# brodeau/aerobulk

Measured on NVIDIA B200. Metric: grid points/s (FP64), higher is better.
Workload: dtype f64

## Files before the change

### aerobulk_b200/csrc/ab_device.cuh

```cuda
#pragma once

#include <cuda_runtime.h>
#include <math.h>

#include "ab_math.cuh"

namespace abd {

#ifndef AB_CS_UNROLL
#define AB_CS_UNROLL 1
#endif
constexpr int CS_UNROLL = AB_CS_UNROLL;
#ifndef AB_PASS_UNROLL
#define AB_PASS_UNROLL 1
#endif
constexpr int PASS_UNROLL = AB_PASS_UNROLL;
#define ABD __device__ __forceinline__
#if defined(AB_NOINLINE) && AB_NOINLINE
#define ABD_HEAVY static __device__ __noinline__
#else
#define ABD_HEAVY __device__ __forceinline__
#endif

template <unsigned long long B>
// ... 274 lines not shown
    } else {
        const PsiMH r = psi_mh_coare_unstable(zeta_u);
        m_u = r.m;
        h_u = r.h;
        if (!ZTEQ) h_t = psi_h_coare_unstable(zeta_t);
    }
}

ABD double cap_zeta(double zeta) { return abm::dmin(abm::dmax(zeta, -50.), 5.); }
ABD PsiMH psi_mh_ecmwf_stable(double zeta)
{
    constexpr double zc = 5. / 0.35;
    const double z = cap_zeta(zeta);
    const double t = KC(2. / 3.) * (z - KC(zc)) * abm::dexp_b(KC(-0.35) * z);
    const double a = fabs(1. + KC(2. / 3.) * z);
    PsiMH r;
    r.m = -t - z - KC(2. / 3. * zc);
    r.h = -t - a * abm::fast_sqrt_pos(a) - KC(2. / 3. * zc) + 1.;
    return r;
}
ABD PsiMH psi_mh_ecmwf_unstable(double zeta)
{
    const double z = cap_zeta(zeta);
    const double x2 = abm::fast_sqrt_pos(fabs(1. - 16. * z));
    const double x = abm::fast_sqrt_pos(x2);
    const double t = 1. + x;
    PsiMH r;
    r.m = abm::dlog(0.125 * t * t * (1. + x2)) - 2. * abm::datan_ge1(x) + KC(0.5 * RPI);
    r.h = 2. * abm::dlog(0.5 * (1. + x2));
    return r;
}
ABD double psi_m_ecmwf_stable(double zeta) { return psi_mh_ecmwf_stable(zeta).m; }
ABD double psi_h_ecmwf_stable(double zeta) { return psi_mh_ecmwf_stable(zeta).h; }
ABD double psi_m_ecmwf_unstable(double zeta) { return psi_mh_ecmwf_unstable(zeta).m; }
ABD double psi_h_ecmwf_unstable(double zeta)
{
    const double x2 = abm::fast_sqrt_pos(fabs(1. - 16. * cap_zeta(zeta)));
    return 2. * abm::dlog(0.5 * (1. + x2));
}

constexpr double ATAN_A_STABLE = 0x1.b53ea749504d7p-1;
constexpr double LOG_A_STABLE = -0x1.ecc2caec5160ap+0;
ABD double psi_m_andreas_stable(double zeta)
{
    const double z = abm::dmin(zeta, 15.);
    constexpr double zam = 5.;
    const double x = abm::fast_cbrt(fabs(1. + z));
    return -(KC(3. * zam / ZBM_A) * (x - 1.))
           + KC(zam * ZBBM_A / (2. * ZBM_A))
                 * (2. * abm::dlog(fabs((x + KC(ZBBM_A)) * KC(1. / (1. + ZBBM_A))))
                    - abm::dlog(fabs((x * x - x * KC(ZBBM_A) + KC(ZBBM_A * ZBBM_A)) * KC(1. / (1. - ZBBM_A + ZBBM_A * ZBBM_A))))
                    + KC(2. * SR3) * (abm::datan_ge1((2. * x - KC(ZBBM_A)) * KC(1. / (SR3 * ZBBM_A))) - KC(ATAN_A_STABLE)));
}
ABD double psi_h_andreas_stable(double zeta)
{
    const double z = abm::dmin(zeta, 15.);
    constexpr double zah = 5., zbh = 5., zch = 3.;
    const double zz = 2. * z + zch;
    return -(KC(0.5 * zbh) * abm::dlog(fabs(1. + zch * z + z * z)))
           + KC(-zah / SR5 + 0.5 * zbh * zch / SR5)
                 * (abm::dlog(fabs(fdiv(zz - KC(SR5), zz + KC(SR5)))) - KC(LOG_A_STABLE));
}
ABD PsiMH psi_mh_andreas_unstable(double zeta)
{
    const double z = abm::dmin(zeta, 15.);
    const double x2 = abm::dmax(abm::fast_sqrt_pos(fabs(1. - 16. * z)), 1.);
    const double x = abm::fast_sqrt_pos(x2);
    PsiMH r;
    const double l2 = abm::dlog(0.5 * (1. + x2));
    r.m = 2. * abm::dlog((1. + x) * 0.5) + l2 - 2. * abm::datan_ge1(x) + KC(RPI * 0.5);
    r.h = 2. * l2;
    return r;
}
ABD double psi_h_andreas_unstable(double zeta)
{
    const double x2 = abm::dmax(abm::fast_sqrt_pos(fabs(1. - 16. * abm::dmin(zeta, 15.))), 1.);
    return 2. * abm::dlog(0.5 * (1. + x2));
}

struct Uniform {
    double zt, zu;
    double log_zt, log_zu, log_ztu, log_zu10, log_10;
    double fg_c_a;
    double fg_1_o_Ribcu;
    double rdt, gdept;
    int nb_iter;
    unsigned long long wl_commit_mask;
    int isd;
    int dawn;
};

struct Guess {
    double us, ts, qs, t_zu, q_zu, Ub, z0;
};

template <bool ZTEQ>
ABD Guess first_guess_coare(const Uniform &u, double sst, double t_zt, double ssq, double q_zt, double wnd, double charn)
{
    Guess g;
    g.t_zu = abm::dmax(t_zt, 180.);
    g.q_zu = abm::dmax(q_zt, 1.e-6);

    double dt = floor_abs(g.t_zu - sst, 1.E-09);
    double dq = floor_abs(g.q_zu - ssq, 1.E-12);

    const double nu_a = visc_air(g.t_zu);
    const double Ub = sqrt(wnd * wnd + 0.5 * 0.5);
    double us = u.fg_c_a * Ub;

    double z0 = charn * us * us * INV_GRAV + fdiv(0.11 * nu_a, us);
    z0 = abm::dmin(abm::dmax(fabs(z0), 1.E-8), 1.);
    const double log_z0 = abm::dlog(z0);

    const double sq = fdiv(VKARMN, u.log_zu - log_z0);
    const double Cd = sq * sq;
    const double r1_o_sqrt_Cd10 = (u.log_10 - log_z0) * INV_VKARMN;

    const double log_z0t = abm::dmin(abm::dmax(u.log_10 - fdiv(VKARMN, 0.00115 * r1_o_sqrt_Cd10), LOG_1EM8), 0.);

    const double Rib = ri_bulk(u.zu, sst, g.t_zu, ssq, g.q_zu, Ub);

    const double cc = fdiv(VKARMN2, Cd * (u.log_zt - log_z0t));
    const double cc_ri = cc * Rib;
    const double zeta_u = nonneg(Rib) ? (cc_ri + 27. / 9. * Rib * Rib) : fdiv(cc_ri, 1. + Rib * u.fg_1_o_Ribcu);

    const double zeta_t = ZTEQ ? zeta_u : fdiv(u.zt * zeta_u, u.zu);
    double psi_m_u, psi_h_u, psi_h_t;
    psi3_coare<ZTEQ>(zeta_u, zeta_t, psi_m_u, psi_h_u, psi_h_t);
    us = abm::dmax(fdiv(Ub * VKARMN, u.log_zu - log_z0 - psi_m_u), 1.E-9);
    const double tmp = fdiv(VKARMN, u.log_zu - log_z0t - psi_h_u);
    double ts = dt * tmp;
    double qs = dq * tmp;

    if (!ZTEQ) {
        const double prf = u.log_ztu + psi_h_u - psi_h_t;
        g.t_zu = t_zt - ts * INV_VKARMN * prf;
        g.q_zu = q_zt - qs * INV_VKARMN * prf;
        g.q_zu = signbit(g.q_zu) ? 0. : g.q_zu;
        dt = floor_abs(g.t_zu - sst, 1.E-09);
        dq = floor_abs(g.q_zu - ssq, 1.E-12);
        ts = dt * tmp;
        qs = dq * tmp;
    }
    g.us = us;
    g.ts = ts;
    g.qs = qs;
    g.Ub = Ub;
    z0 = charn * us * us * INV_GRAV + fdiv(0.11 * nu_a, us);
    g.z0 = abm::dmin(abm::dmax(fabs(z0), 1.E-8), 1.);
    return g;
}

template <bool COARE_FORM>
ABD double cool_skin_dT(double alpha, double Qsw, double Qnsol, double us, double Qlat)
{
    const double usw = abm::dmax(us, KC(1.E-4)) * KC(SQ_RADRW);
    const double usw2 = usw * usw;
    const double c_lamb = fdiv(alpha * KC(RCST_CS), usw2 * usw2);
    const double nu_o_usw = fdiv(KC(RNU0_W), usw);
    const double d_warm = abm::dmin(6. * nu_o_usw, KC(0.007));
    const double q_lat_term = COARE_FORM ? fdiv(KC(0.026) * abm::dmin(Qlat, 0.) * KC(RCP0_W * (1. / RLEVAP)), alpha) : 0.;

    auto delta = [&](double Qd) -> double {
        const double zQd = COARE_FORM ? Qd + q_lat_term : Qd;
        if (nonneg(zQd)) return d_warm;
        const double x = abm::dmax(c_lamb * zQd, KC(1.e-30));
        const double x75 = abm::pow075_pos(x);
        return 6. * abm::fast_rcbrt(1. + x75) * nu_o_usw;
    };

    double Qabs = Qnsol, d = 0.;
#pragma unroll CS_UNROLL
    for (int jc = 0; jc < 5; ++jc) {
        const double d_prev = d;
        if (jc > 0) {
            const double fr = abm::dmax((COARE_FORM ? KC(0.137) : KC(0.065)) + 11. * d - fdiv(KC(6.6E-5), d) * (1. - abm::dexp(-d * KC(1. / 8.E-4))), KC(0.01));
            Qabs = Qnsol + fr * Qsw;
        }
        d = delta(Qabs);
        if (jc > 0 && d == d_prev) break;
    }
    return Qabs * d * KC(1. / RK0_W);
}

struct WarmLayer {
    double dT, Hz, Qac, Tac;
};

struct WlCoareCtx {
    double cd1, cd2;
    bool dawn;
};
__host__ __device__ inline bool wl_coare_dawn(double lon, int isd)
{
    auto f_mod = [](double a, double p) {
        double r = fmod(a, p);
        if (r != 0. && ((r < 0.) != (p < 0.))) r += p;
        return r;
    };
    double lag = -1. * f_mod((360. - f_mod(lon, 360.)) / 15., 24.);
    lag = -1. * copysign(fmin(fabs(lag), fabs(f_mod(lag, 24.))), lag + 12.);
    const int ilag = (int)(lag * 3600.);
    int isol = (isd + ilag) % 86400;
    if (isol < 0) isol += 86400;
    const double hr = (double)isol / 3600.;
    return (hr > 4.) && (hr <= 6.5);
}
ABD WlCoareCtx wl_coare_ctx(double alpha, bool dawn)
{
    WlCoareCtx c;
    c.dawn = dawn;
    const double Rich0 = 0.65;
    c.cd1 = sqrt(2. * Rich0 * RCP0_W / (alpha * GRAV * RHO0_W));
    c.cd2 = sqrt(2. * alpha * GRAV / (Rich0 * RHO0_W)) / RCP0W_POW15;
    return c;
}
ABD double wl_coare_absorption(double H)
{
    const double e1 = (H > KC(0.53)) ? 0. : abm::dexp_b(-H * KC(1. / 0.014));
    const double e2 = (H > KC(13.4)) ? 0. : abm::dexp_b(-H * KC(1. / 0.357));
    return 1. - fdiv(KC(0.28 * 0.014) * (1. - e1) + KC(0.27 * 0.357) * (1. - e2)
                     + KC(0.45 * 12.82) * (1 - abm::dexp_b(-H * KC(1. / 12.82))), H);
}
ABD void wl_coare(WarmLayer &w, const WlCoareCtx &c, double Qsw, double Qnsol, double Tau, double rdt,
                  double gdept, bool commit)
{
    const double Hwl_max = 20.;
    double dT = w.dT;
    double H = abm::dmax(abm::dmin(w.Hz, Hwl_max), 0.1);
    double qac = w.Qac;
    double tac = w.Tac;
    bool l_exit = c.dawn, destroy = c.dawn;
    double Qabs = 0.;

    if (!l_exit) {
        Qabs = wl_coare_absorption(H) * Qsw + Qnsol;
        if (fabs(dT) < 1.E-6 && Qabs <= 0.) l_exit = true;
    }
    if (!l_exit && (w.Qac + Qabs * rdt <= 0.)) {
        l_exit = true;
        destroy = true;
    }
    if (!l_exit) {
        tac = w.Tac + abm::dmax(.002, Tau) * rdt;
#pragma unroll 1
        for (int jl = 0; jl < 5; ++jl) {
            if (jl > 0) Qabs = wl_coare_absorption(H) * Qsw + Qnsol;
            qac = w.Qac + Qabs * rdt;
            if (qac <= 0.) break;
            const double H_prev = H;
            H = abm::dmax(abm::dmin(Hwl_max, c.cd1 * tac * abm::fast_rsqrt(qac)), 0.1);
            if (H == H_prev) break;
        }
        if (qac <= 0.) {
            destroy = true;
        } else {
            dT = fdiv(c.cd2 * (qac * (qac * abm::fast_rsqrt(qac))), tac);
            if (signbit(gdept - H)) dT = dT * fdiv(gdept, H);
        }
    }
    if (destroy) {
        dT = 0.;
        H = Hwl_max;
        qac = 0.;
        tac = 0.;
    }
    if (commit) {
        w.dT = dT;
        w.Hz = H;
        w.Qac = qac;
        w.Tac = tac;
    }
}

ABD double phi_takaya(double z)
{
    const double z2 = z * z;
    if (nonneg(z)) return 1. + fdiv(5. * z + 4. * z2, 1. + 3. * z + 0.25 * z2);
    return abm::fast_rsqrt(1. - 16. * (-fabs(z)));
}
struct WlEcmwfCtx {
    double fr, tcorr, r_tcorr;
};
ABD WlEcmwfCtx wl_ecmwf_ctx(double H, double gdept)
{
    WlEcmwfCtx c;
    c.tcorr = signbit(gdept - H) ? gdept / H : 1.;
    c.r_tcorr = 1. / c.tcorr;
    c.fr = 1. - 0.28 * abm::dexp(-71.5 * H) - 0.27 * abm::dexp(-2.8 * H) - 0.45 * abm::dexp(-0.07 * H);
    return c;
}
ABD void wl_ecmwf(WarmLayer &w, const WlEcmwfCtx &c, double alpha, double Qsw, double Qnsol, double us, double rdt)
{
    const double rNuwl0 = 0.5;
    const double RhoCp_w = RHO0_W * RCP0_W;
    const double H = w.Hz;
    const double tcorr = c.tcorr;
    const double dT_b = abm::dmax(w.dT * c.r_tcorr, 0.);

    const double Qabs = c.fr * Qsw + Qnsol;

    const double usw = abm::dmax(us, KC(1.E-4)) * KC(SQ_RADRW);
    const double usw2 = usw * usw;
    const bool warming = nonneg(Qabs);

    const double cst1 = KC(VKARMN * GRAV) * alpha;
    const double L2 = fdiv(cst1 * Qabs, RhoCp_w * usw2 * usw);
    const double cst2 = fdiv(cst1, 5. * H * usw2);
    const double cst0 = fdiv(rdt * (rNuwl0 + 1.), H);
    const double A = cst0 * Qabs * KC(1. / (rNuwl0 * RhoCp_w));
    const double cst3 = -cst0 * KC(VKARMN) * usw * KC(FLA_ECMWF);

    const double B_warm = warming ? fdiv(cst3, phi_takaya(H * L2)) : 0.;
    double dT_n = dT_b;
#pragma unroll 2
    for (int jc = 0; jc < 10; ++jc) {
        const double prev = dT_n;
        dT_n = 0.5 * (dT_n + dT_b);
        const double B = warming ? B_warm : fdiv(cst3, phi_takaya(H * abm::fast_sqrt(dT_n * cst2)));
        dT_n = abm::dmax(dT_b + A + B * dT_n, 0.);
        if (dT_n == prev) break;
    }
    w.dT = dT_n * tcorr;
}

struct PointIn {
    double sst, theta_zt, ssq, q_zt, wnd, slp;
    double Qsw, rlw, lon;
    bool has_lon;
};
struct Coeffs {
    double Cd, Ch, Ce, t_zu, q_zu, Ub, Ts, qs;
};
struct Diag {
    double CdN, ChN, CeN, z0, us, L, UN10, dT_cs;
};

ABD double cd_n10_ncar(double w)
{
    double w6 = w * w * w;
    w6 = w6 * w6;
    const double r = nonneg(w - 33.) ? KC(1.e-3 * 2.34)
                                     : KC(1.e-3) * (fdiv(KC(2.7), w) + KC(0.142) + w * KC(1. / 13.09) - KC(3.14807E-10) * w6);
    return abm::dmax(r, KC(CX_MIN));
}

template <bool ZTEQ>
ABD Coeffs solve_ncar(const Uniform &u, const PointIn &p, Diag &dg)
{
    const double Ub = abm::dmax(0.5, p.wnd);
    const bool stable0 = nonneg(virt_temp(p.theta_zt, p.q_zt) - virt_temp(p.sst, p.ssq));
    double CdN = cd_n10_ncar(Ub);
    double sqrt_CdN = abm::fast_sqrt_pos(CdN);
    double Cd = CdN;
    double Ce = abm::dmax(1.e-3 * (34.6 * sqrt_CdN), CX_MIN);
    double Ch = abm::dmax(1.e-3 * sqrt_CdN * (stable0 ? 18. : 32.7), CX_MIN);
    double sqrt_Cd = sqrt_CdN;
    double t_zu = abm::dmax(p.theta_zt, 180.);
    double q_zu = abm::dmax(p.q_zt, 1.e-6);
    double us = 0., r1oL = 0., Un10 = 0., ChN = 0., CeN = 0.;

#pragma unroll 1
    for (int jit = 0; jit < u.nb_iter; ++jit) {
        const double dt = t_zu - p.sst;
        const double dq = q_zu - p.ssq;
        us = sqrt_Cd * Ub;
        const double r_sqrt_Cd = abm::fast_rcp(sqrt_Cd);
        const double ts = Ch * r_sqrt_Cd * dt;
        const double qs = Ce * r_sqrt_Cd * dq;
        r1oL = one_on_L(t_zu, q_zu, us, ts, qs);
        const double zeta_u = clip_abs(u.zu * r1oL, 10.);
        const double zeta_t = clip_abs(u.zt * r1oL, 10.);
        double psi_m, psi_h_u, psi_h_t = 0.;
        if (nonneg(zeta_u)) {
            psi_m = psi_h_u = -5. * zeta_u;
            if (!ZTEQ) psi_h_t = -5. * zeta_t;
        } else {
            const PsiMH r = psi_mh_ncar_unstable(zeta_u);
            psi_m = r.m;
            psi_h_u = r.h;
            if (!ZTEQ) psi_h_t = psi_h_ncar_unstable(zeta_t);
        }
        if (!ZTEQ) {
            const double tmp = u.log_ztu + psi_h_u - psi_h_t;
            t_zu = p.theta_zt - ts * INV_VKARMN * tmp;
            q_zu = abm::dmax(0., p.q_zt - qs * INV_VKARMN * tmp);
        }
        Un10 = abm::dmax(0.25, sqrt_Cd * Ub * INV_VKARMN * (VKARMN * r_sqrt_Cd + psi_m - u.log_zu10));
        CdN = cd_n10_ncar(Un10);
        sqrt_CdN = abm::fast_sqrt_pos(CdN);
        double tmp = 1. + sqrt_CdN * INV_VKARMN * (u.log_zu10 - psi_m);
        Cd = abm::dmax(fdiv(CdN, tmp * tmp), CX_MIN);
        sqrt_Cd = abm::fast_sqrt_pos(Cd);
        const double r_sqrt_CdN = abm::fast_rcp(sqrt_CdN);
        tmp = (u.log_zu10 - psi_h_u) * INV_VKARMN * r_sqrt_CdN;
        const double tmp2 = sqrt_Cd * r_sqrt_CdN;
        ChN = 1.e-3 * sqrt_CdN * (nonneg(zeta_u) ? 18. : 32.7);
        CeN = 1.e-3 * (34.6 * sqrt_CdN);
        Ch = abm::dmax(fdiv(ChN * tmp2, 1. + ChN * tmp), CX_MIN);
        Ce = abm::dmax(fdiv(CeN * tmp2, 1. + CeN * tmp), CX_MIN);
    }
    Coeffs c;
    c.Cd = Cd; c.Ch = Ch; c.Ce = Ce; c.t_zu = t_zu; c.q_zu = q_zu; c.Ub = Ub; c.Ts = p.sst; c.qs = p.ssq;
    dg.CdN = CdN; dg.ChN = ChN; dg.CeN = CeN; dg.UN10 = Un10; dg.L = 1. / r1oL; dg.us = us;
    dg.z0 = abm::dmin(u.zu * abm::dexp_b(-VKARMN * abm::fast_rsqrt(CdN)), Z0_SEA_MAX);
    dg.dT_cs = 0.;
    return c;
}

ABD double charn_coare3p0(double w)
{
    if (!nonneg(w - 10.)) return 0.011;
    if (nonneg(w - 18.)) return 0.018;
    return 0.011 + (0.018 - 0.011) * (w - 10.) * (1. / (18. - 10.));
}
ABD double charn_coare3p6(double w) { return abm::dmax(abm::dmin(KC(0.0017) * w - KC(0.005), KC(0.028)), 0.); }

template <bool V36, bool CS, bool WL, bool ZTEQ>
ABD Coeffs solve_coare(const Uniform &u, const PointIn &p, WarmLayer &wl, Diag &dg)
{
    constexpr bool SKIN = CS || WL;
    constexpr double zi0 = 600., Beta0 = V36 ? 1.2 : 1.25, zeta_abs_max = 50.;

    double Ts = p.sst, qs_ = p.ssq;
    double alpha = 0.;
    WlCoareCtx wc = {};
    if (SKIN) {
        if (CS) Ts = Ts - 0.25;
        qs_ = RDCT_QSAT_SALT * q_sat(abm::dmax(Ts, 200.), p.slp);
        alpha = alpha_sw(p.sst);
        if (WL) wc = wl_coare_ctx(alpha, p.has_lon ? wl_coare_dawn(p.lon, u.isd) : (u.dawn != 0));
    }

    const Guess g = first_guess_coare<ZTEQ>(u, Ts, p.theta_zt, qs_, p.q_zt, p.wnd,
                                            V36 ? charn_coare3p6(p.wnd) : charn_coare3p0(p.wnd));
    double us = g.us, ts = g.ts, qst = g.qs, t_zu = g.t_zu, q_zu = g.q_zu, Ub = g.Ub;
    double log_z0 = abm::dlog(g.z0);
    const double nu_a = V36 ? visc_air(t_zu) : visc_air(p.theta_zt);

    double dt = floor_abs(t_zu - Ts, 1.E-09);
    double dq = floor_abs(q_zu - qs_, 1.E-12);
    double dT_cs = 0., r1oL = 0., z0 = g.z0, log_z0t = 0.;

#pragma unroll 1
    for (int jit = 1; jit <= u.nb_iter; ++jit) {
        const double us2 = us * us;
        r1oL = one_on_L(t_zu, q_zu, us, ts, qst);

        const double cv = abm::fast_cbrt(abm::dmax(KC(-zi0 * INV_VKARMN) * r1oL, 0.));
        const double gust2 = KC(Beta0 * Beta0) * us2 * (cv * cv);
        Ub = abm::dmax(abm::fast_sqrt(p.wnd * p.wnd + gust2), KC(0.2));

        const double zeta_u = clip_abs(u.zu * r1oL, zeta_abs_max);

        const double Un10 = us * INV_VKARMN * (u.log_10 - log_z0);
        const double r_us = abm::fast_rcp(us);
        z0 = (V36 ? charn_coare3p6(Un10) : charn_coare3p0(Un10)) * us2 * KC(INV_GRAV) + KC(0.11) * nu_a * r_us;
        z0 = abm::dmin(abm::dmax(fabs(z0), KC(1.E-9)), 1.);
        log_z0 = abm::dlog(z0);

        const double log_rr = abm::dlog(nu_a * r_us) - log_z0;
        log_z0t = V36 ? abm::dmax(abm::dmin(KC(LOG_1P6EM4), KC(LOG_5P8EM5) + KC(0.72) * log_rr), KC(LOG_1EM9))
                      : abm::dmax(abm::dmin(KC(LOG_1P1EM4), KC(LOG_5P5EM5) + KC(0.6) * log_rr), KC(LOG_1EM9));

        const double zeta_t = clip_abs(u.zt * r1oL, zeta_abs_max);
        double psi_m_u, psi_h_u, psi_h_t;
        psi3_coare<ZTEQ>(zeta_u, zeta_t, psi_m_u, psi_h_u, psi_h_t);
        double tmp1 = fdiv(KC(VKARMN), u.log_zu - log_z0t - psi_h_u);
        ts = dt * tmp1;
        qst = dq * tmp1;
        us = abm::dmax(fdiv(Ub * KC(VKARMN), u.log_zu - log_z0 - psi_m_u), KC(1.E-9));

        if (!ZTEQ) {
            tmp1 = u.log_zt - u.log_zu + psi_h_u - psi_h_t;
            t_zu = p.theta_zt - ts * INV_VKARMN * tmp1;
            q_zu = p.q_zt - qst * INV_VKARMN * tmp1;
        } else if (!V36) {
            t_zu = p.theta_zt;
            q_zu = p.q_zt;
        }

        if (SKIN) {
            const AirZu air = air_at_zu(u.zu, t_zu, q_zu, p.slp);
            const bool commit = (jit < 64) ? ((u.wl_commit_mask >> jit) & 1ull) != 0ull : (u.nb_iter % jit) == 0;
#pragma unroll PASS_UNROLL
            for (int pass = CS ? 0 : 1; pass < (WL ? 2 : 1); ++pass) {
                const double Ts_q = Ts;
                if (CS && pass == 0) {
                    double Qns, Tau, Qlat;
                    update_qnsol_tau(air, Ts, qs_, t_zu, q_zu, us, ts, qst, p.wnd, Ub, p.rlw, Qns, Tau, Qlat);
                    dT_cs = cool_skin_dT<true>(alpha, p.Qsw, Qns, us, Qlat);
                    Ts = p.sst + dT_cs;
                    if (WL) Ts = Ts + wl.dT;
                } else {
                    if (commit) {
                        double Qns, Tau, Qlat;
                        update_qnsol_tau(air, Ts, qs_, t_zu, q_zu, us, ts, qst, p.wnd, Ub, p.rlw, Qns, Tau, Qlat);
                        wl_coare(wl, wc, p.Qsw, Qns, Tau, u.rdt, u.gdept, true);
                    }
                    Ts = p.sst + wl.dT;
                    if (CS) Ts = Ts + dT_cs;
                }
                if (Ts != Ts_q) qs_ = KC(RDCT_QSAT_SALT) * q_sat(abm::dmax(Ts, 200.), p.slp);
            }
        }
        if (SKIN || !ZTEQ || !V36) {
            dt = floor_abs(t_zu - Ts, KC(1.E-09));
            dq = floor_abs(q_zu - qs_, KC(1.E-12));
        }
    }
    Coeffs c;
    const double r = fdiv(us, Ub);
    c.Cd = abm::dmax(r * r, CX_MIN);
    c.Ch = abm::dmax(fdiv(r * ts, dt), CX_MIN);
    c.Ce = abm::dmax(fdiv(r * qst, dq), CX_MIN);
    c.t_zu = t_zu; c.q_zu = q_zu; c.Ub = Ub; c.Ts = Ts; c.qs = qs_;
    const double t0 = 1. / (u.log_zu - log_z0);
    dg.CdN = abm::dmax(VKARMN2 * t0 * t0, CX_MIN);
    dg.ChN = dg.CeN = abm::dmax(VKARMN2 * t0 / (u.log_zu - log_z0t), CX_MIN);
    dg.z0 = z0; dg.us = us; dg.L = 1. / r1oL; dg.UN10 = us * INV_VKARMN * (u.log_10 - log_z0);
    dg.dT_cs = dT_cs;
    return c;
}

template <bool CS, bool WL, bool ZTEQ>
ABD Coeffs solve_ecmwf(const Uniform &u, const PointIn &p, WarmLayer &wl, Diag &dg)
{
    constexpr bool SKIN = CS || WL;
    constexpr double charn0 = 0.018, zi0 = 1000., Beta0 = 1., alpha_M = 0.11, alpha_H = 0.40, alpha_Q = 0.62;

    double Ts = p.sst, qs_ = p.ssq;
    double alpha = 0.;
    WlEcmwfCtx wec = {};
    if (SKIN) {
        if (CS) Ts = Ts - 0.25;
        qs_ = RDCT_QSAT_SALT * q_sat(abm::dmax(Ts, 200.), p.slp);
        alpha = alpha_sw(p.sst);
        if (WL) wec = wl_ecmwf_ctx(wl.Hz, u.gdept);
    }

    const Guess g = first_guess_coare<ZTEQ>(u, Ts, p.theta_zt, qs_, p.q_zt, p.wnd, charn0);
    double us = g.us, ts = g.ts, qst = g.qs, t_zu = g.t_zu, q_zu = g.q_zu, Ub = g.Ub;
    double z0 = g.z0;
    double log_z0 = abm::dlog(z0);
    const double nu_a = visc_air(p.theta_zt);

    double dt = floor_abs(t_zu - Ts, 1.E-09);
    double dq = floor_abs(q_zu - qs_, 1.E-12);

    double r1oL = one_on_L(t_zu, q_zu, us, ts, qst);
    const double x0 = fdiv(VKARMN, fdiv(0.00115, fdiv(VKARMN, u.log_10 - log_z0)));
    double z0t = abm::dmin(abm::dmax(10. * abm::dexp(-x0), 1.E-9), 1.);
    double log_z0t = abm::dmin(abm::dmax(u.log_10 - x0, LOG_1EM9), 0.);

    double Fm, Fh, psi_h_u;
    if (nonneg(r1oL)) {
        const PsiMH pu = psi_mh_ecmwf_stable(u.zu * r1oL);
        psi_h_u = pu.h;
        Fm = u.log_zu - log_z0 - pu.m + psi_m_ecmwf_stable(z0 * r1oL);
        Fh = u.log_zu - log_z0t - psi_h_u + psi_h_ecmwf_stable(z0t * r1oL);
    } else {
        const PsiMH pu = psi_mh_ecmwf_unstable(u.zu * r1oL);
        psi_h_u = pu.h;
        Fm = u.log_zu - log_z0 - pu.m + psi_m_ecmwf_unstable(z0 * r1oL);
        Fh = u.log_zu - log_z0t - psi_h_u + psi_h_ecmwf_unstable(z0t * r1oL);
    }
    double log_z0q = 0., psi_h_z0q = 0., dT_cs = 0.;

#pragma unroll 1
    for (int jit = 1; jit <= u.nb_iter; ++jit) {
        const double Rib = ri_bulk(u.zu, Ts, t_zu, qs_, q_zu, Ub);
        r1oL = clip_abs(fdiv(Rib * Fm * Fm, Fh * u.zu), 200.);

        const bool stable = nonneg(r1oL);
        double psi_m_u, psi_h_t = 0., psi_m_z0old;
        if (stable) {
            const PsiMH pu = psi_mh_ecmwf_stable(u.zu * r1oL);
            psi_m_u = pu.m;
            psi_h_u = pu.h;
            if (!ZTEQ) psi_h_t = psi_h_ecmwf_stable(u.zt * r1oL);
            psi_m_z0old = psi_m_ecmwf_stable(z0 * r1oL);
        } else {
            const PsiMH pu = psi_mh_ecmwf_unstable(u.zu * r1oL);
            psi_m_u = pu.m;
            psi_h_u = pu.h;
            if (!ZTEQ) psi_h_t = psi_h_ecmwf_unstable(u.zt * r1oL);
            psi_m_z0old = psi_m_ecmwf_unstable(z0 * r1oL);
        }

        Fm = u.log_zu - log_z0 - psi_m_u + psi_m_z0old;

        us = fdiv(Ub * KC(VKARMN), Fm);
        const double us2 = us * us;
        double tmp0 = fdiv(nu_a, us);
        z0 = abm::dmin(fabs(KC(alpha_M) * tmp0 + KC(charn0) * us2 * KC(INV_GRAV)), KC(0.001));
        z0t = abm::dmin(fabs(KC(alpha_H) * tmp0), KC(0.001));
        const double z0q = abm::dmin(fabs(KC(alpha_Q) * tmp0), KC(0.001));
        log_z0 = abm::dlog(z0);
        const double log_t0 = abm::dlog(fabs(tmp0));
        log_z0t = abm::dmin(KC(LOG_0P40) + log_t0, KC(LOG_1EM3));
        log_z0q = abm::dmin(KC(LOG_0P62) + log_t0, KC(LOG_1EM3));

        double psi_m_z0, psi_h_z0t;
        if (stable) {
            psi_m_z0 = psi_m_ecmwf_stable(z0 * r1oL);
            psi_h_z0t = psi_h_ecmwf_stable(z0t * r1oL);
            psi_h_z0q = psi_h_ecmwf_stable(z0q * r1oL);
        } else {
            psi_m_z0 = psi_m_ecmwf_unstable(z0 * r1oL);
            psi_h_z0t = psi_h_ecmwf_unstable(z0t * r1oL);
            psi_h_z0q = psi_h_ecmwf_unstable(z0q * r1oL);
        }

        const double cv = abm::fast_cbrt(abm::dmax(-zi0 * r1oL * INV_VKARMN, 0.));
        tmp0 = Beta0 * Beta0 * us2 * (cv * cv);
        Ub = abm::dmax(abm::fast_sqrt(p.wnd * p.wnd + tmp0), KC(0.2));

        tmp0 = psi_h_u - psi_h_z0t;
        double tmp1 = fdiv(KC(VKARMN), u.log_zu - log_z0t - tmp0);
        ts = dt * tmp1;
        if (!ZTEQ) {
            tmp1 = u.log_ztu + tmp0 - psi_h_t + psi_h_z0t;
            t_zu = p.theta_zt - ts * INV_VKARMN * tmp1;
        } else {
            t_zu = p.theta_zt;
        }
        tmp0 = psi_h_u - psi_h_z0q;
        tmp1 = fdiv(KC(VKARMN), u.log_zu - log_z0q - tmp0);
        qst = dq * tmp1;
        if (!ZTEQ) {
            tmp1 = u.log_ztu + tmp0 - psi_h_t + psi_h_z0q;
            q_zu = abm::dmax(p.q_zt - qst * INV_VKARMN * tmp1, 0.);
        } else {
            q_zu = abm::dmax(p.q_zt, 0.);
        }

        Fm = u.log_zu - log_z0 - psi_m_u + psi_m_z0;
        Fh = u.log_zu - log_z0t - psi_h_u + psi_h_z0t;

        if (SKIN) {
            const AirZu air = air_at_zu(u.zu, t_zu, q_zu, p.slp);
#pragma unroll PASS_UNROLL
            for (int pass = CS ? 0 : 1; pass < (WL ? 2 : 1); ++pass) {
                double Qns, Tau, Qlat;
                update_qnsol_tau(air, Ts, qs_, t_zu, q_zu, us, ts, qst, p.wnd, Ub, p.rlw, Qns, Tau, Qlat);
                if (CS && pass == 0) {
                    dT_cs = cool_skin_dT<false>(alpha, p.Qsw, Qns, us, 0.);
                    Ts = p.sst + dT_cs;
                    if (WL) Ts = Ts + wl.dT;
                } else {
                    wl_ecmwf(wl, wec, alpha, p.Qsw, Qns, us, u.rdt);
                    Ts = p.sst + wl.dT;
                    if (CS) Ts = Ts + dT_cs;
                }
                qs_ = KC(RDCT_QSAT_SALT) * q_sat(abm::dmax(Ts, 200.), p.slp);
            }
        }
        dt = floor_abs(t_zu - Ts, KC(1.E-09));
        dq = floor_abs(q_zu - qs_, KC(1.E-12));
    }
    Coeffs c;
    const double Fq = u.log_zu - log_z0q - psi_h_u + psi_h_z0q;
    const double k2_o_Fm = fdiv(VKARMN2, Fm);
    c.Cd = abm::dmax(fdiv(k2_o_Fm, Fm), CX_MIN);
    c.Ch = abm::dmax(fdiv(k2_o_Fm, Fh), CX_MIN);
    c.Ce = abm::dmax(fdiv(k2_o_Fm, Fq), CX_MIN);
    c.t_zu = t_zu; c.q_zu = q_zu; c.Ub = Ub; c.Ts = Ts; c.qs = qs_;
    const double t0 = 1. / (u.log_zu - log_z0);
    dg.CdN = abm::dmax(VKARMN2 * t0 * t0, CX_MIN);
    dg.ChN = dg.CeN = abm::dmax(VKARMN2 * t0 / (u.log_zu - log_z0t), CX_MIN);
    dg.z0 = z0; dg.us = us; dg.L = 1. / r1oL; dg.UN10 = us * INV_VKARMN * (u.log_10 - log_z0);
    dg.dT_cs = dT_cs;
    return c;
}

template <bool ZTEQ>
ABD Coeffs solve_andreas(const Uniform &u, const PointIn &p, Diag &dg)
{
    const double rRi_max = 0.15, rCs_min = 0.35E-3;
    const double Ub = abm::dmax(0.25, p.wnd);
    const double r_Ub = abm::fast_rcp(Ub);
    double UN10 = Ub;
    double t_zu = p.theta_zt, q_zu = p.q_zt;
    const double sq0 = sqrt(1.1E-3);
    double t_star = 1.1E-3 / sq0 * (t_zu - p.sst);
    double q_star = 1.1E-3 / sq0 * (q_zu - p.ssq);
    double RiB = ri_bulk(u.zu, p.sst, t_zu, p.ssq, q_zu, Ub);
    double u_star = 0., zeta_u = 0., z0 = 0., psi_m = 0.;

#pragma unroll 1
    for (int jit = 1; jit <= u.nb_iter; ++jit) {
        if (RiB < rRi_max) {
            const double za = UN10 - KC(8.271);
            u_star = KC(0.239) + KC(0.0433) * (za + abm::fast_sqrt_pos(KC(0.12) * za * za + KC(0.181)));
        } else {
            u_star = KC(0x1.47ae147ae147bp-7) * Ub;
        }
        zeta_u = u.zu * one_on_L(t_zu, q_zu, u_star, t_star, q_star);
        const double r = u_star * r_Ub;
        const double Cd = abm::dmax(r * r, CX_MIN);
        const double zeta_t = fdiv(zeta_u, u.zu) * u.zt;
        const bool adjust = !ZTEQ && jit > 1;
        double psi_h_u, psi_h_t = 0.;
        if (nonneg(abm::dmin(zeta_u, 15.))) {
            psi_m = psi_m_andreas_stable(zeta_u);
            psi_h_u = psi_h_andreas_stable(zeta_u);
            if (adjust) psi_h_t = psi_h_andreas_stable(zeta_t);
        } else {
            const PsiMH r = psi_mh_andreas_unstable(zeta_u);
            psi_m = r.m;
            psi_h_u = r.h;
            if (adjust) psi_h_t = psi_h_andreas_unstable(zeta_t);
        }
        const double log_z0 = abm::dmin(u.log_zu - (VKARMN * abm::fast_rsqrt(Cd) + psi_m), LOG_Z0_SEA_MAX);
        z0 = abm::dexp(log_z0);

        const double Rer = fdiv(z0 * u_star, visc_air(t_zu));
        const double log_Rer = abm::dlog(abm::dmax(Rer, 1.E-300));
        const double log_z0t = log_z0tq_LKB(1, Rer, log_Rer, log_z0);
        const double log_z0q = log_z0tq_LKB(2, Rer, log_Rer, log_z0);

        t_star = fdiv((t_zu - p.sst) * VKARMN, u.log_zu - log_z0t - psi_h_u);
        q_star = fdiv((q_zu - p.ssq) * VKARMN, u.log_zu - log_z0q - psi_h_u);

        if (adjust) {
            const double tmp = u.log_ztu + psi_h_u - psi_h_t;
            t_zu = p.theta_zt - t_star * INV_VKARMN * tmp;
            q_zu = p.q_zt - q_star * INV_VKARMN * tmp;
            RiB = ri_bulk(u.zu, p.sst, t_zu, p.ssq, q_zu, Ub);
        }
        UN10 = abm::dmax(0.1, Ub - u_star * INV_VKARMN * (u.log_zu10 - psi_m));
    }
    Coeffs c;
    const double r = u_star * r_Ub;
    c.Cd = abm::dmax(r * r, CX_MIN);
    const double d1 = floor_abs(t_zu - p.sst, 1.E-6);
    const double d2 = floor_abs(q_zu - p.ssq, 1.E-9);
    c.Ch = abm::dmax(fdiv(r * t_star, d1), rCs_min);
    c.Ce = abm::dmax(fdiv(r * q_star, d2), rCs_min);
    c.t_zu = t_zu; c.q_zu = q_zu; c.Ub = Ub; c.Ts = p.sst; c.qs = p.ssq;
    const double log_z0 = abm::dlog(z0);
    const double t0 = 1. / (u.log_zu - log_z0);
    dg.CdN = abm::dmax(VKARMN2 * t0 * t0, CX_MIN);
    const double Rer = z0 * u_star / visc_air(t_zu);
    const double log_Rer = abm::dlog(abm::dmax(Rer, 1.E-300));
    dg.ChN = VKARMN2 * t0 / (u.log_zu - log_z0tq_LKB(1, Rer, log_Rer, log_z0));
    dg.CeN = VKARMN2 * t0 / (u.log_zu - log_z0tq_LKB(2, Rer, log_Rer, log_z0));
    dg.z0 = z0; dg.us = u_star; dg.L = u.zu / zeta_u;
    dg.UN10 = Ub - u_star * INV_VKARMN * (u.log_zu10 - psi_m);
    dg.dT_cs = 0.;
    return c;
}

template <int ALGO, bool CS, bool WL, bool ZTEQ>
ABD Coeffs solve_ocean(const Uniform &u, const PointIn &p, WarmLayer &wl, Diag &dg)
{
    if (ALGO == NCAR) return solve_ncar<ZTEQ>(u, p, dg);
    else if (ALGO == ANDREAS) return solve_andreas<ZTEQ>(u, p, dg);
    else if (ALGO == ECMWF) return solve_ecmwf<CS, WL, ZTEQ>(u, p, wl, dg);
    else return solve_coare<ALGO == COARE3P6, CS, WL, ZTEQ>(u, p, wl, dg);
}

#undef ABD
}
```

### aerobulk_b200/csrc/ab_kernels.cu

```cuda
#include "ab_kernels.cuh"

#include <float.h>
#include <stdint.h>

namespace abk {

using namespace abd;

#ifndef AB_FLUX_BLOCK
#define AB_FLUX_BLOCK 256
#endif
#ifndef AB_MIN_BLOCKS
#define AB_MIN_BLOCKS 3
#endif
#ifndef AB_MIN_BLOCKS_NOSKIN
#define AB_MIN_BLOCKS_NOSKIN 4
#endif
static constexpr int FLUX_BLOCK = AB_FLUX_BLOCK;

#ifndef AB_SORT_BAND
#define AB_SORT_BAND 0.15
#endif
#ifndef AB_SORT_BAND_SKIN
#define AB_SORT_BAND_SKIN 0.5
#endif
#ifndef AB_SORT_BAND_NOQ
#define AB_SORT_BAND_NOQ 1.0
#endif
template <class T>
__device__ __forceinline__ double ld(const void *p, long long i) { return (double)__ldg(static_cast<const T *>(p) + i); }
template <class T>
__device__ __forceinline__ void st(void *p, long long i, double v) { static_cast<T *>(p)[i] = v; }
template <>
__device__ __forceinline__ void st<float>(void *p, long long i, double v) { static_cast<float *>(p)[i] = __double2float_rn(v); }

template <class T>
__device__ __forceinline__ float stability_proxy(const FluxArgs &a, int ihum, double skin_off, long long i)
{
    const double sst = ld<T>(a.sst, i) + skin_off, ta = ld<T>(a.t_zt, i) + RGAMMA_DRY * a.u.zt;
    const float d0 = (float)(ta - sst);
    if (ihum != 0) return d0;
    const float q = (float)ld<T>(a.hum_zt, i), p = (float)ld<T>(a.slp, i);
    const float tc = (float)(sst - 273.15);
    const float es = 611.2f * __expf(17.67f * tc * __frcp_rn(tc + 243.5f));
    const float qs = 0.98f * 0.622f * es * __frcp_rn(p - 0.378f * es);
    return d0 + 0.608f * ((float)ta * q - (float)sst * qs);
}

static constexpr int SORT_WIN = 2048;
static constexpr int SORT_BLOCK = 256;
static constexpr int SORT_ITEMS = SORT_WIN / SORT_BLOCK;
static constexpr int SORT_CLASSES = 3;

template <class T>
__device__ __forceinline__ void classify_block(const FluxArgs &a, unsigned short *perm, int skin, int tid)
{
    constexpr int NW = SORT_BLOCK / 32, NG = SORT_ITEMS * NW;
    __shared__ unsigned short s_c[SORT_CLASSES][NG], s_off[SORT_CLASSES][NG];
    __shared__ int s_tot[SORT_CLASSES];
    const long long base = (long long)blockIdx.x * SORT_WIN;
    const int lane = tid & 31, w = tid >> 5;
    const int ihum = a.init_dev ? __ldg(a.init_dev) : a.ihum;
    const float band = (ihum != 0) ? (float)AB_SORT_BAND_NOQ : (skin ? (float)AB_SORT_BAND_SKIN : (float)AB_SORT_BAND);
    const bool wl = skin && !a.first_step && a.dT_wl != nullptr;
    int cls[SORT_ITEMS];
#pragma unroll
    for (int k = 0; k < SORT_ITEMS; ++k) {
        const long long i = base + k * SORT_BLOCK + tid;
        cls[k] = SORT_CLASSES;
        if (i < a.n) {
            const double off = skin ? (-0.25 + (wl ? a.dT_wl[i] : 0.)) : 0.;
            const float d = stability_proxy<T>(a, ihum, off, i);
            cls[k] = (d >= band) ? 0 : (d > -band) ? 1 : 2;
        }
    }
    const unsigned lt = (1u << lane) - 1u;
    int rank[SORT_ITEMS], real_rank[SORT_ITEMS];
#pragma unroll
    for (int k = 0; k < SORT_ITEMS; ++k) {
        unsigned any = 0u;
        rank[k] = 0;
#pragma unroll
        for (int c = 0; c < SORT_CLASSES; ++c) {
            const unsigned b = __ballot_sync(0xffffffffu, cls[k] == c);
            if (lane == 0) s_c[c][k * NW + w] = (unsigned short)__popc(b);
            if (cls[k] == c) rank[k] = __popc(b & lt);
            any |= b;
        }
        real_rank[k] = __popc(any & lt);
    }
    __syncthreads();
    static_assert(NG == 64 && SORT_CLASSES * 32 <= SORT_BLOCK, "prefix layout");
    if (w < SORT_CLASSES) {
        const int a0 = s_c[w][2 * lane], a1 = s_c[w][2 * lane + 1];
        int incl = a0 + a1;
#pragma unroll
        for (int o = 1; o < 32; o <<= 1) {
            const int t = __shfl_up_sync(0xffffffffu, incl, o);
            if (lane >= o) incl += t;
        }
        const int excl = incl - (a0 + a1);
        s_off[w][2 * lane] = (unsigned short)excl;
        s_off[w][2 * lane + 1] = (unsigned short)(excl + a0);
        if (lane == 31) s_tot[w] = incl;
    }
    __syncthreads();
    const int tot0 = s_tot[0], tot1 = s_tot[1], tot2 = s_tot[2];
#pragma unroll
    for (int k = 0; k < SORT_ITEMS; ++k) {
        const int g = k * NW + w, item = k * SORT_BLOCK + tid;
        int slot;
        if (cls[k] < SORT_CLASSES) {
            const int before = (cls[k] > 0 ? tot0 : 0) + (cls[k] > 1 ? tot1 : 0);
            slot = before + s_off[cls[k]][g] + rank[k];
        } else {
            const int real_before = s_off[0][g] + s_off[1][g] + s_off[2][g] + real_rank[k];
            slot = tot0 + tot1 + tot2 + (item - real_before);
        }
        perm[base + slot] = (unsigned short)item;
    }
}

__global__ void __launch_bounds__(SORT_BLOCK) classify_kernel(const FluxArgs a, unsigned short *perm, int skin)
{
    classify_block<double>(a, perm, skin, threadIdx.x);
}

template <class T>
__global__ void __launch_bounds__(SORT_BLOCK) classify_io_kernel(const FluxArgs a, unsigned short *perm, int skin)
{
    classify_block<T>(a, perm, skin, threadIdx.x);
}

template <int ALGO, class Args>
__device__ __forceinline__ void load_warm_layer(const Args &a, long long i, WarmLayer &wl)
{
    if (ALGO == ECMWF) {
        wl.Hz = 3.;
        wl.dT = a.first_step ? 0. : a.dT_wl[i];
    } else if (a.first_step) {
        wl.Hz = 20.;
    } else {
        wl.dT = a.dT_wl[i];
        wl.Hz = a.Hz_wl[i];
        wl.Qac = a.Qnt_ac[i];
        wl.Tac = a.Tau_ac[i];
    }
}
template <int ALGO, class Args>
__device__ __forceinline__ void store_warm_layer(const Args &a, long long i, const WarmLayer &wl)
{
    a.dT_wl[i] = wl.dT;
    if (ALGO != ECMWF) {
        a.Hz_wl[i] = wl.Hz;
        a.Qnt_ac[i] = wl.Qac;
        a.Tau_ac[i] = wl.Tac;
    }
}

template <class T, int ALGO, bool SKIN, bool ZTEQ>
__device__ __forceinline__ void flux_point(const FluxArgs &a, unsigned tid)
{
    abm::load_tables();
    long long i = (long long)blockIdx.x * FLUX_BLOCK + tid;
    if (a.perm) i = (i / SORT_WIN) * SORT_WIN + a.perm[i];
    if (i >= a.n) return;
    int ihum = a.ihum;
    if (a.init_dev) {
        if (__ldg(a.init_dev + 1) != 0) return;
        ihum = __ldg(a.init_dev);
    }

    const double sst = ld<T>(a.sst, i);
    const double t_air = ld<T>(a.t_zt, i);
    const double hum = ld<T>(a.hum_zt, i);
    const double U = ld<T>(a.U_zu, i);
    const double V = ld<T>(a.V_zu, i);
    const double slp = ld<T>(a.slp, i);

    PointIn p;
    p.sst = sst;
    p.slp = slp;
    if (ihum == 0) p.q_zt = hum;
    else if (ihum == 1) p.q_zt = q_air_dp(hum, abm::dmax(slp, 50000.));
    else p.q_zt = q_air_rh(hum, t_air, abm::dmax(slp, 50000.));
    p.wnd = sqrt(__dadd_rn(__dmul_rn(U, U), __dmul_rn(V, V)));
    p.ssq = RDCT_QSAT_SALT * q_sat(sst, slp);
    p.theta_zt = theta_from_z_P0_T_q(a.u.zt, slp, t_air, p.q_zt);
    p.Qsw = 0.;
    p.rlw = 0.;
    p.lon = 0.;
    p.has_lon = false;

    WarmLayer wl = {0., 0., 0., 0.};
    if (SKIN) {
        p.Qsw = (1. - ROCE_ALB0) * ld<T>(a.rad_sw, i);
        p.rlw = ld<T>(a.rad_lw, i);
        if (a.lon) {
            p.lon = __ldg(a.lon + i);
            p.has_lon = true;
        }
        load_warm_layer<ALGO>(a, i, wl);
    }

    Diag dg;
    const Coeffs c = solve_ocean<ALGO, SKIN, SKIN, ZTEQ>(a.u, p, wl, dg);
    if (SKIN) store_warm_layer<ALGO>(a, i, wl);

    const Flux f = bulk_formula(air_at_zu(a.u.zu, c.t_zu, c.q_zu, slp), c.Ts, c.qs, c.t_zu, c.q_zu, c.Cd, c.Ch, c.Ce, p.wnd, c.Ub);
    if (f.tau > REF_TAU_MAX) atomicMin(a.bad_index, (unsigned long long)(a.index_offset + i));

    double tx = 0., ty = 0.;
    if (p.wnd > 1.E-3) {
        const double s = f.tau / p.wnd;
        tx = s * U;
        ty = s * V;
    }
    st<T>(a.QL, i, f.qlat);
    st<T>(a.QH, i, f.qsen);
    st<T>(a.Tau_x, i, tx);
    st<T>(a.Tau_y, i, ty);
    st<T>(a.Evap, i, f.evap);
    if (a.T_s) st<T>(a.T_s, i, c.Ts);
}

template <int ALGO, bool SKIN, bool ZTEQ>
__global__ void __launch_bounds__(FLUX_BLOCK, SKIN ? AB_MIN_BLOCKS : AB_MIN_BLOCKS_NOSKIN) flux_kernel(const FluxArgs a)
{
    flux_point<double, ALGO, SKIN, ZTEQ>(a, threadIdx.x);
}

template <class T, int ALGO, bool SKIN, bool ZTEQ>
__global__ void __launch_bounds__(FLUX_BLOCK, SKIN ? AB_MIN_BLOCKS : AB_MIN_BLOCKS_NOSKIN) flux_io_kernel(const FluxArgs a)
{
    flux_point<T, ALGO, SKIN, ZTEQ>(a, threadIdx.x);
}

static auto flux_kernel_for(int algo, bool skin, bool zteq, size_t elem = ELEM_F64)
{
    return pick_ocean(algo, skin, zteq, [elem](auto A, auto S, auto Z) {
        return elem == ELEM_F64 ? flux_kernel<A(), S(), Z()> : elem == ELEM_F32 ? flux_io_kernel<float, A(), S(), Z()> : nullptr;
    });
}

cudaError_t launch_flux(int algo, bool skin, bool zteq, size_t elem, const FluxArgs &a, cudaStream_t s)
{
    const auto k = flux_kernel_for(algo, skin, zteq, elem);
    if (!k) return cudaErrorInvalidValue;
    if (a.n <= 0) return cudaSuccess;
    const long long span = a.perm ? (a.n + SORT_WIN - 1) / SORT_WIN * SORT_WIN : a.n;
    k<<<(unsigned)((span + FLUX_BLOCK - 1) / FLUX_BLOCK), FLUX_BLOCK, 0, s>>>(a);
    return cudaGetLastError();
}

template <int ALGO, bool CS, bool WL, bool ZTEQ>
__global__ void __launch_bounds__(FLUX_BLOCK, (CS || WL) ? AB_MIN_BLOCKS : AB_MIN_BLOCKS_NOSKIN) turb_kernel(const TurbArgs a)
{
    abm::load_tables();
    const long long i = (long long)blockIdx.x * FLUX_BLOCK + threadIdx.x;
    if (i >= a.n) return;
    constexpr bool SKIN = CS || WL;
    PointIn p;
    p.sst = a.T_s[i];
    p.ssq = a.q_s[i];
    p.theta_zt = __ldg(a.t_zt + i);
    p.q_zt = __ldg(a.q_zt + i);
    p.wnd = __ldg(a.U_zu + i);
    p.slp = 0.;
    p.Qsw = 0.;
    p.rlw = 0.;
    p.lon = 0.;
    p.has_lon = false;
    WarmLayer wl = {0., 0., 0., 0.};
    if (SKIN) {
        p.Qsw = __ldg(a.Qsw + i);
        p.rlw = __ldg(a.rad_lw + i);
        p.slp = __ldg(a.slp + i);
        if (a.lon) {
            p.lon = __ldg(a.lon + i);
            p.has_lon = true;
        }
    }
    if (WL) load_warm_layer<ALGO>(a, i, wl);
    Diag dg;
    const Coeffs c = solve_ocean<ALGO, CS, WL, ZTEQ>(a.u, p, wl, dg);
    if (WL) store_warm_layer<ALGO>(a, i, wl);
    if (SKIN) {
        a.T_s[i] = c.Ts;
        a.q_s[i] = c.qs;
    }
    a.Cd[i] = c.Cd; a.Ch[i] = c.Ch; a.Ce[i] = c.Ce;
    a.t_zu[i] = c.t_zu; a.q_zu[i] = c.q_zu; a.Ubzu[i] = c.Ub;
    if (a.opt[0]) a.opt[0][i] = dg.CdN;
    if (a.opt[1]) a.opt[1][i] = dg.ChN;
    if (a.opt[2]) a.opt[2][i] = dg.CeN;
    if (a.opt[3]) a.opt[3][i] = dg.z0;
    if (a.opt[4]) a.opt[4][i] = dg.us;
    if (a.opt[5]) a.opt[5][i] = dg.L;
    if (a.opt[6]) a.opt[6][i] = dg.UN10;
    if (CS && a.opt[7]) a.opt[7][i] = dg.dT_cs;
    if (WL && a.opt[8]) a.opt[8][i] = wl.dT;
    if (WL && a.opt[9]) a.opt[9][i] = wl.Hz;
}

cudaError_t launch_turb(int algo, bool cs, bool wl, bool zteq, const TurbArgs &a, cudaStream_t s)
{
    const auto k = pick_ocean(algo, cs || wl, zteq, [cs, wl](auto A, auto S, auto Z) {
        if constexpr (!S()) return turb_kernel<A(), false, false, Z()>;
        else return cs ? (wl ? turb_kernel<A(), true, true, Z()> : turb_kernel<A(), true, false, Z()>)
                       : turb_kernel<A(), false, true, Z()>;
    });
    if (!k) return cudaErrorInvalidValue;
    if (a.n <= 0) return cudaSuccess;
    k<<<(unsigned)((a.n + FLUX_BLOCK - 1) / FLUX_BLOCK), FLUX_BLOCK, 0, s>>>(a);
    return cudaGetLastError();
}

int flux_block_size() { return FLUX_BLOCK; }

int sort_window() { return SORT_WIN; }

cudaError_t launch_classify(size_t elem, const FluxArgs &a, unsigned short *perm, bool skin, cudaStream_t s)
{
    const auto k = elem == ELEM_F64 ? classify_kernel : elem == ELEM_F32 ? classify_io_kernel<float> : nullptr;
    if (!k) return cudaErrorInvalidValue;
    if (a.n <= 0) return cudaSuccess;
    const long long nwin = (a.n + SORT_WIN - 1) / SORT_WIN;
    k<<<(unsigned)nwin, SORT_BLOCK, 0, s>>>(a, perm, skin ? 1 : 0);
    return cudaGetLastError();
}

cudaError_t flux_kernel_attributes(int algo, bool skin, bool zteq, cudaFuncAttributes *attr, int *blocks_per_sm)
{
    const auto k = flux_kernel_for(algo, skin, zteq);
    if (!k) return cudaErrorInvalidValue;
    cudaError_t e = cudaFuncGetAttributes(attr, k);
    if (e != cudaSuccess || !blocks_per_sm) return e;
    return cudaOccupancyMaxActiveBlocksPerMultiprocessor(blocks_per_sm, k, FLUX_BLOCK, 0);
}

static constexpr int STATS_BLOCK = 256;
static constexpr int STATS_MAX_BLOCKS = 148 * 8;

__device__ __forceinline__ bool point_unmasked(double sst, double ta, double slp, double wnd, bool rad, double rlw)
{
    bool m = true;
    if (sst < 270. || sst > 320.) m = false;
    if (ta < 180. || ta > 330.) m = false;
    if (slp < 80000. || slp > 110000.) m = false;
    if (wnd > 50.) m = false;
    if (rad) {
        if (rlw < 0. || rlw > 1500.) m = false;
        if (rlw < 0. || rlw > 750.) m = false;
    }
    return m;
}

__device__ __forceinline__ double warp_reduce(double v, int op)
{
// ... 397 lines not shown
```

Before: 4.295 billion.

## Compact divergent skin-layer iterations across block via shared-memory work queue

For skin-enabled kernels, threads that need the expensive cool-skin or warm-layer iterative solve are ballot-collected per block. When they are spread sparsely across warps, their inputs go to shared memory and the work is redistributed so that fewer warps execute it densely. This aims to cut warp divergence in the iterative skin loops. In exchange it adds block-wide syncthreads, about 18KB of shared memory per block that may lower occupancy, and out-of-range threads must stay alive to take part in the barriers.

Result: slower. 4.037 billion (median of 6 runs) (-6.0%).

```diff
diff --git a/aerobulk_b200/csrc/ab_device.cuh b/aerobulk_b200/csrc/ab_device.cuh
--- a/aerobulk_b200/csrc/ab_device.cuh
+++ b/aerobulk_b200/csrc/ab_device.cuh
@@ -450,6 +450,16 @@
 }
 
 template <bool COARE_FORM>
+ABD double cool_skin_qlat_term(double alpha, double Qlat)
+{
+    return COARE_FORM ? fdiv(KC(0.026) * abm::dmin(Qlat, 0.) * KC(RCP0_W * (1. / RLEVAP)), alpha) : 0.;
+}
+template <bool COARE_FORM>
+ABD bool cool_skin_cools(double alpha, double Qnsol, double Qlat)
+{
+    return !nonneg(COARE_FORM ? Qnsol + cool_skin_qlat_term<COARE_FORM>(alpha, Qlat) : Qnsol);
+}
+template <bool COARE_FORM>
 ABD double cool_skin_dT(double alpha, double Qsw, double Qnsol, double us, double Qlat)
 {
     const double usw = abm::dmax(us, KC(1.E-4)) * KC(SQ_RADRW);
@@ -457,7 +467,7 @@
     const double c_lamb = fdiv(alpha * KC(RCST_CS), usw2 * usw2);
     const double nu_o_usw = fdiv(KC(RNU0_W), usw);
     const double d_warm = abm::dmin(6. * nu_o_usw, KC(0.007));
-    const double q_lat_term = COARE_FORM ? fdiv(KC(0.026) * abm::dmin(Qlat, 0.) * KC(RCP0_W * (1. / RLEVAP)), alpha) : 0.;
+    const double q_lat_term = cool_skin_qlat_term<COARE_FORM>(alpha, Qlat);
 
     auto delta = [&](double Qd) -> double {
         const double zQd = COARE_FORM ? Qd + q_lat_term : Qd;
@@ -570,6 +580,13 @@
         w.Tac = tac;
     }
 }
+ABD bool wl_coare_iterates(const WarmLayer &w, const WlCoareCtx &c, double Qsw, double Qnsol, double rdt)
+{
+    if (c.dawn) return false;
+    const double Qabs = wl_coare_absorption(abm::dmax(abm::dmin(w.Hz, 20.), 0.1)) * Qsw + Qnsol;
+    if (fabs(w.dT) < 1.E-6 && Qabs <= 0.) return false;
+    return !(w.Qac + Qabs * rdt <= 0.);
+}
 
 ABD double phi_takaya(double z)
 {
@@ -621,6 +638,26 @@
     }
     w.dT = dT_n * tcorr;
 }
+ABD bool wl_ecmwf_cools(const WarmLayer &w, const WlEcmwfCtx &c, double Qsw, double Qnsol)
+{
+    return !nonneg(c.fr * Qsw + Qnsol) && w.dT * c.r_tcorr > 0.;
+}
+
+struct SkinInline {
+    template <bool COARE_FORM>
+    ABD double cool_skin(double alpha, double Qsw, double Qnsol, double us, double Qlat) const
+    {
+        return cool_skin_dT<COARE_FORM>(alpha, Qsw, Qnsol, us, Qlat);
+    }
+    ABD void warm_coare(WarmLayer &w, const WlCoareCtx &c, double Qsw, double Qnsol, double Tau, double rdt, double gdept) const
+    {
+        wl_coare(w, c, Qsw, Qnsol, Tau, rdt, gdept, true);
+    }
+    ABD void warm_ecmwf(WarmLayer &w, const WlEcmwfCtx &c, double alpha, double Qsw, double Qnsol, double us, double rdt) const
+    {
+        wl_ecmwf(w, c, alpha, Qsw, Qnsol, us, rdt);
+    }
+};
 
 struct PointIn {
     double sst, theta_zt, ssq, q_zt, wnd, slp;
@@ -714,8 +751,8 @@
 }
 ABD double charn_coare3p6(double w) { return abm::dmax(abm::dmin(KC(0.0017) * w - KC(0.005), KC(0.028)), 0.); }
 
-template <bool V36, bool CS, bool WL, bool ZTEQ>
-ABD Coeffs solve_coare(const Uniform &u, const PointIn &p, WarmLayer &wl, Diag &dg)
+template <bool V36, bool CS, bool WL, bool ZTEQ, class Skin>
+ABD Coeffs solve_coare(const Uniform &u, const PointIn &p, WarmLayer &wl, Diag &dg, const Skin &sk)
 {
     constexpr bool SKIN = CS || WL;
     constexpr double zi0 = 600., Beta0 = V36 ? 1.2 : 1.25, zeta_abs_max = 50.;
@@ -787,14 +824,14 @@
                 if (CS && pass == 0) {
                     double Qns, Tau, Qlat;
                     update_qnsol_tau(air, Ts, qs_, t_zu, q_zu, us, ts, qst, p.wnd, Ub, p.rlw, Qns, Tau, Qlat);
-                    dT_cs = cool_skin_dT<true>(alpha, p.Qsw, Qns, us, Qlat);
+                    dT_cs = sk.template cool_skin<true>(alpha, p.Qsw, Qns, us, Qlat);
                     Ts = p.sst + dT_cs;
                     if (WL) Ts = Ts + wl.dT;
                 } else {
                     if (commit) {
                         double Qns, Tau, Qlat;
                         update_qnsol_tau(air, Ts, qs_, t_zu, q_zu, us, ts, qst, p.wnd, Ub, p.rlw, Qns, Tau, Qlat);
-                        wl_coare(wl, wc, p.Qsw, Qns, Tau, u.rdt, u.gdept, true);
+                        sk.warm_coare(wl, wc, p.Qsw, Qns, Tau, u.rdt, u.gdept);
                     }
                     Ts = p.sst + wl.dT;
                     if (CS) Ts = Ts + dT_cs;
@@ -821,8 +858,8 @@
     return c;
 }
 
-template <bool CS, bool WL, bool ZTEQ>
-ABD Coeffs solve_ecmwf(const Uniform &u, const PointIn &p, WarmLayer &wl, Diag &dg)
+template <bool CS, bool WL, bool ZTEQ, class Skin>
+ABD Coeffs solve_ecmwf(const Uniform &u, const PointIn &p, WarmLayer &wl, Diag &dg, const Skin &sk)
 {
     constexpr bool SKIN = CS || WL;
     constexpr double charn0 = 0.018, zi0 = 1000., Beta0 = 1., alpha_M = 0.11, alpha_H = 0.40, alpha_Q = 0.62;
@@ -943,11 +980,11 @@
                 double Qns, Tau, Qlat;
                 update_qnsol_tau(air, Ts, qs_, t_zu, q_zu, us, ts, qst, p.wnd, Ub, p.rlw, Qns, Tau, Qlat);
                 if (CS && pass == 0) {
-                    dT_cs = cool_skin_dT<false>(alpha, p.Qsw, Qns, us, 0.);
+                    dT_cs = sk.template cool_skin<false>(alpha, p.Qsw, Qns, us, 0.);
                     Ts = p.sst + dT_cs;
                     if (WL) Ts = Ts + wl.dT;
                 } else {
-                    wl_ecmwf(wl, wec, alpha, p.Qsw, Qns, us, u.rdt);
+                    sk.warm_ecmwf(wl, wec, alpha, p.Qsw, Qns, us, u.rdt);
                     Ts = p.sst + wl.dT;
                     if (CS) Ts = Ts + dT_cs;
                 }
@@ -1050,13 +1087,13 @@
     return c;
 }
 
-template <int ALGO, bool CS, bool WL, bool ZTEQ>
-ABD Coeffs solve_ocean(const Uniform &u, const PointIn &p, WarmLayer &wl, Diag &dg)
+template <int ALGO, bool CS, bool WL, bool ZTEQ, class Skin = SkinInline>
+ABD Coeffs solve_ocean(const Uniform &u, const PointIn &p, WarmLayer &wl, Diag &dg, const Skin &sk = Skin())
 {
     if (ALGO == NCAR) return solve_ncar<ZTEQ>(u, p, dg);
     else if (ALGO == ANDREAS) return solve_andreas<ZTEQ>(u, p, dg);
-    else if (ALGO == ECMWF) return solve_ecmwf<CS, WL, ZTEQ>(u, p, wl, dg);
-    else return solve_coare<ALGO == COARE3P6, CS, WL, ZTEQ>(u, p, wl, dg);
+    else if (ALGO == ECMWF) return solve_ecmwf<CS, WL, ZTEQ>(u, p, wl, dg, sk);
+    else return solve_coare<ALGO == COARE3P6, CS, WL, ZTEQ>(u, p, wl, dg, sk);
 }
 
 #undef ABD
diff --git a/aerobulk_b200/csrc/ab_kernels.cu b/aerobulk_b200/csrc/ab_kernels.cu
--- a/aerobulk_b200/csrc/ab_kernels.cu
+++ b/aerobulk_b200/csrc/ab_kernels.cu
@@ -158,13 +158,128 @@
     }
 }
 
+static constexpr int SKQ_FIELDS = 9;
+static constexpr int SKQ_WARPS = FLUX_BLOCK / 32;
+struct SkinQueueSmem {
+    double v[SKQ_FIELDS][FLUX_BLOCK];
+    unsigned mask[2][SKQ_WARPS];
+};
+
+struct SkinBlockQueue {
+    SkinQueueSmem &s;
+    unsigned tid;
+    mutable unsigned call = 0;
+
+    template <class Work>
+    __device__ __forceinline__ bool run(bool queued, Work work) const
+    {
+        const unsigned *mask = s.mask[call++ & 1u];
+        const unsigned m = __ballot_sync(0xffffffffu, queued);
+        if ((tid & 31) == 0) s.mask[(call - 1u) & 1u][tid >> 5] = m;
+        __syncthreads();
+        int total = 0, busy = 0;
+#pragma unroll
+        for (int w = 0; w < SKQ_WARPS; ++w) {
+            const int c = __popc(mask[w]);
+            total += c;
+            busy += (c != 0);
+        }
+        if ((total + 31) / 32 >= busy) return false;
+        int k = tid, w = 0;
+#pragma unroll 1
+        for (; w < SKQ_WARPS; ++w) {
+            const int c = __popc(mask[w]);
+            if (k < c) break;
+            k -= c;
+        }
+        if (w < SKQ_WARPS) work(32 * w + (int)__fns(mask[w], 0, k + 1));
+        __syncthreads();
+        return true;
+    }
+
+    template <bool COARE_FORM>
+    __device__ __forceinline__ double cool_skin(double alpha, double Qsw, double Qnsol, double us, double Qlat) const
+    {
+        const bool queued = cool_skin_cools<COARE_FORM>(alpha, Qnsol, Qlat);
+        if (queued) {
+            s.v[0][tid] = alpha;
+            s.v[1][tid] = Qsw;
+            s.v[2][tid] = Qnsol;
+            s.v[3][tid] = us;
+            s.v[4][tid] = Qlat;
+        }
+        if (run(queued, [&](int o) { s.v[0][o] = cool_skin_dT<COARE_FORM>(s.v[0][o], s.v[1][o], s.v[2][o], s.v[3][o], s.v[4][o]); })
+            && queued)
+            return s.v[0][tid];
+        return cool_skin_dT<COARE_FORM>(alpha, Qsw, Qnsol, us, Qlat);
+    }
+
+    __device__ __forceinline__ void put(int o, const WarmLayer &w) const
+    {
+        s.v[0][o] = w.dT;
+        s.v[1][o] = w.Hz;
+        s.v[2][o] = w.Qac;
+        s.v[3][o] = w.Tac;
+    }
+    __device__ __forceinline__ WarmLayer get(int o) const { return WarmLayer{s.v[0][o], s.v[1][o], s.v[2][o], s.v[3][o]}; }
+
+    __device__ __forceinline__ void warm_coare(WarmLayer &w, const WlCoareCtx &c, double Qsw, double Qnsol, double Tau,
+                                               double rdt, double gdept) const
+    {
+        const bool queued = wl_coare_iterates(w, c, Qsw, Qnsol, rdt);
+        if (queued) {
+            put(tid, w);
+            s.v[4][tid] = c.cd1;
+            s.v[5][tid] = c.cd2;
+            s.v[6][tid] = Qsw;
+            s.v[7][tid] = Qnsol;
+            s.v[8][tid] = Tau;
+        }
+        if (run(queued, [&](int o) {
+                WarmLayer q = get(o);
+                wl_coare(q, WlCoareCtx{s.v[4][o], s.v[5][o], false}, s.v[6][o], s.v[7][o], s.v[8][o], rdt, gdept, true);
+                put(o, q);
+            }) && queued)
+            w = get(tid);
+        else
+            wl_coare(w, c, Qsw, Qnsol, Tau, rdt, gdept, true);
+    }
+
+    __device__ __forceinline__ void warm_ecmwf(WarmLayer &w, const WlEcmwfCtx &c, double alpha, double Qsw, double Qnsol,
+                                               double us, double rdt) const
+    {
+        const bool queued = wl_ecmwf_cools(w, c, Qsw, Qnsol);
+        if (queued) {
+            s.v[0][tid] = w.dT;
+            s.v[1][tid] = w.Hz;
+            s.v[2][tid] = c.fr;
+            s.v[3][tid] = c.tcorr;
+            s.v[4][tid] = c.r_tcorr;
+            s.v[5][tid] = alpha;
+            s.v[6][tid] = Qsw;
+            s.v[7][tid] = Qnsol;
+            s.v[8][tid] = us;
+        }
+        if (run(queued, [&](int o) {
+                WarmLayer q = {s.v[0][o], s.v[1][o], 0., 0.};
+                wl_ecmwf(q, WlEcmwfCtx{s.v[2][o], s.v[3][o], s.v[4][o]}, s.v[5][o], s.v[6][o], s.v[7][o], s.v[8][o], rdt);
+                s.v[0][o] = q.dT;
+            }) && queued)
+            w.dT = s.v[0][tid];
+        else
+            wl_ecmwf(w, c, alpha, Qsw, Qnsol, us, rdt);
+    }
+};
+
 template <class T, int ALGO, bool SKIN, bool ZTEQ>
 __device__ __forceinline__ void flux_point(const FluxArgs &a, unsigned tid)
 {
     abm::load_tables();
     long long i = (long long)blockIdx.x * FLUX_BLOCK + tid;
     if (a.perm) i = (i / SORT_WIN) * SORT_WIN + a.perm[i];
-    if (i >= a.n) return;
+    const bool live = i < a.n;
+    if (SKIN ? !__syncthreads_or(live) : !live) return;
+    if (!live) i = a.n - 1;
     int ihum = a.ihum;
     if (a.init_dev) {
         if (__ldg(a.init_dev + 1) != 0) return;
@@ -204,7 +319,14 @@
     }
 
     Diag dg;
-    const Coeffs c = solve_ocean<ALGO, SKIN, SKIN, ZTEQ>(a.u, p, wl, dg);
+    Coeffs c;
+    if constexpr (SKIN) {
+        __shared__ SkinQueueSmem skq;
+        c = solve_ocean<ALGO, SKIN, SKIN, ZTEQ>(a.u, p, wl, dg, SkinBlockQueue{skq, tid});
+    } else {
+        c = solve_ocean<ALGO, SKIN, SKIN, ZTEQ>(a.u, p, wl, dg);
+    }
+    if (!live) return;
     if (SKIN) store_warm_layer<ALGO>(a, i, wl);
 
     const Flux f = bulk_formula(air_at_zu(a.u.zu, c.t_zu, c.q_zu, slp), c.Ts, c.qs, c.t_zu, c.q_zu, c.Cd, c.Ch, c.Ce, p.wnd, c.Ub);
```
